# open-speech/HTK

Hardware: AMD Instinct MI355X
Metric: herest_gmm_frame_state_loglik_per_sec (higher is better)
Workload: dtype f32 (scores: bf16x3 split operands, fp32 accumulate) + f64 (alpha / beta with fp32-transcendental log-add, accumulators); 1 GPU; HERest EM iteration (pass + accumulator all-reduce + model update), 5000 tied states x 16 mix, D=39, 1250 x 500-frame utterances per GPU (BASELINE config[2]: 10k utterances sharded 8-way); states=5000, mix=16, utts_per_gpu=1250, frames=500, chunks=1, update=HERest -m 3 -v 0.01, on the device

## Files before the change

### htk_amd/csrc/fb.hip

```cpp
#include <hip/hip_runtime.h>
#include <cstdio>
#include <cstdlib>
#include <cstring>
#include <cmath>
#include <algorithm>
#include <vector>
#include <thread>
#include <mutex>
#include <condition_variable>
#include <functional>
#include "internal.h"
#include "hipcheck.h"
#include "kernels.h"
#include "devbuf.h"

static constexpr char fbOwner[] = "fb";
typedef DevBufT<fbOwner> DevBuf;

struct PrepPool {
   std::vector<std::thread> th;
   std::mutex mu;
   std::condition_variable cvGo, cvDone;
   std::function<void(int)> job;
   int generation = 0, pending = 0, nJobs = 0;
// ... 105 lines not shown

struct ResLayout {
   size_t nUtt;
   size_t status() const { return sizeof(double) * nUtt; }
   size_t counter() const { return (sizeof(double) + sizeof(int)) * nUtt; }
   size_t flag() const { return counter() + sizeof(int); } size_t bytes() const { return counter() + 2 * sizeof(int); }
};

enum { UTT_NO_TEE = 1, UTT_ALL_LR = 2 };

struct htkamd_fb : BatchTables {
   htkamd_model *m = nullptr;
   int nUtt = 0;
   int debug = 0;
   int forceGeneral = 0;
   int noStatePath = 0;
   int noLrPath = 0;
   int topoVersion = 0;
   std::vector<unsigned char> uttFlags;
   UttClasses cls;
   size_t gamTotal = 0, betaWTotal = 0, alphaWTotal = 0;
   int totalFrames = 0, nCellsMax = 1, QMax = 1, TMax = 1, blockDim = 64;
   long long frameStates = 0;
   const float *dX = nullptr;
   DevBuf d_arena;
   DevBuf d_qLo, d_qHi, d_aLo, d_aHi, d_outp, d_beta, d_gam, d_alpha, d_pr;
   DevBuf d_betaW;
   DevBuf d_tmE, d_tmMaxP;
   DevBuf d_outpU;
   DevBuf d_alphaW, d_qBeam, d_aBeam, d_trPart, d_hits, d_hitCtl;
   DevBuf d_sink;
   DevBuf d_stCnt, d_stBucket;
   DevBuf d_laneRec;
   bool mixStateLast = false;
   bool mixDeferred = false;
   FbArgs *faMix = nullptr;
   const int *qBeamLast = nullptr;
   DevBuf d_transOff, d_trOccOff, d_counter;
   DevBuf d_rec, d_recSorted, d_recCtl;
   int recCapForce = 0;
   PrepPool *pool = nullptr; std::vector<PrepChunk> *chunks = nullptr;
   void *h_arena = nullptr; size_t h_arenaCap = 0;
   void *h_res = nullptr; size_t h_resCap = 0;
   hipEvent_t evRes = nullptr; bool resPending = false;
   bool f16Pass = false;
   hipEvent_t ev[6] = {}, evK[2] = {}, evCopy = nullptr;
   hipStream_t resStream = nullptr;
   bool timed = false, copyPending = false, scored = false;
   int evMode = 0, evModeLast = 0;
   ResLayout res() const { return {(size_t)nUtt}; }
};

static bool compat_revisit(const htkamd_model *m) { return (m->compat & HTKAMD_COMPAT_STREAM_REVISIT) && m->NSt > 1 && m->NSt != 3 && !m->tiedMix; }

extern "C" int htkamd_fb_create(htkamd_model *m, htkamd_fb **out)
{
   if (!m || !out) { htkamd_set_error("fb_create: NULL argument"); return HTKAMD_EINVAL; }
   if (m->fullc) { htkamd_set_error("fb_create: forward-backward on FULLC models is not supported yet (its mixture statistics are diagonal)"); return HTKAMD_EMODEL; }
   if (m->maxM > 4096) { htkamd_set_error("fb_create: %d mixture components per state not supported", m->maxM); return HTKAMD_EMODEL; }
   htkamd_fb *fb = new htkamd_fb();
   fb->m = m;
   auto fail = [&](const char *what, hipError_t e) { htkamd_set_error("fb_create: %s: %s", what, hipGetErrorString(e)); htkamd_fb_destroy(fb); return HTKAMD_EHIP; };
   hipError_t e;
   for (hipEvent_t *v : {&fb->ev[0], &fb->ev[1], &fb->ev[2], &fb->ev[3], &fb->ev[4], &fb->ev[5], &fb->evK[0], &fb->evK[1]})
      if ((e = hipEventCreate(v)) != hipSuccess) return fail("hipEventCreate", e);
   if ((e = hipEventCreateWithFlags(&fb->evCopy, hipEventDisableTiming)) != hipSuccess) return fail("hipEventCreate", e);
// ... 424 lines not shown
   fa.mN = fb->mN.dev; fa.mTp = fb->mTp.dev; fa.mCell0 = fb->mCell0.dev; fa.mSlot0 = fb->mSlot0.dev; fa.mDms = fb->mDms.dev; fa.mHmm = fb->mHmm.dev; fa.mTrans = fb->mTrans.dev;
   fa.sQ = fb->sQ.dev; fa.thrCell = fb->thrCell.dev; fa.cQ = fb->cQ.dev; fa.cI = fb->cI.dev; fa.slotState = fb->slotState.dev;
   fa.taperLo = fb->taperLo.dev; fa.taperHi = fb->taperHi.dev;
   fa.qLo = (short *)fb->d_qLo.p; fa.qHi = (short *)fb->d_qHi.p; fa.aLo = (short *)fb->d_aLo.p; fa.aHi = (short *)fb->d_aHi.p;
   fa.X = fb->dX; fa.transP = m->d_transP; fa.outp = (float *)fb->d_outp.p;
   fa.beta = (double *)fb->d_beta.p; fa.gam = (double *)fb->d_gam.p; fa.alphaDbg = fb->debug ? (double *)fb->d_alpha.p : nullptr;
   fa.pr = (double *)fb->d_pr.p; fa.status = (int *)((char *)fb->d_pr.p + fb->res().status());
   fa.stateCompOff = m->d_stateCompOff; fa.compGauss = m->d_compGauss;
   fa.NSt = m->NSt; fa.outpU = (const float *)fb->d_outpU.p; fa.dimStream = m->d_dimStream;
   fa.compatRevisit = compat_revisit(m) && !fb->nextSame.empty(); fa.nextSame = fb->nextSame.dev;
   fa.transOff = (const int *)fb->d_transOff.p; fa.trOccOff = (const int *)fb->d_trOccOff.p;
   fa.compLogWt = m->d_compLogWt; fa.gparam = m->d_gparam; fa.mean = m->d_mean; fa.laddTab = m->d_laddTab;
   fa.PS = m->PS; fa.D = m->D; fa.maxN = m->maxN; fa.maxM = m->maxM;
   fa.nCellsMax = fb->nCellsMax; fa.QMax = fb->QMax; fa.TMax = fb->TMax;
   fa.acc = accs->d_vec; fa.lay = accs->lay;
   fa.pruneInit = cfg->pruneInit; fa.pruneInc = cfg->pruneInc; fa.pruneLim = cfg->pruneLim;
   fa.minLogExp = m->minLogExp; fa.minFrwdP = cfg->minFrwdP; fa.uFlags = cfg->uFlags;
   fa.gamTotal = fb->gamTotal; fa.gamOffByUtt = fb->gamOff.dev; fa.gamChunkUtt = fb->gamChunkUtt.dev;
   return fa;
}

struct LdsSizes { size_t beta, alpha; };
static LdsSizes fb_lds_sizes(const FbArgs &fa)
{
   const size_t nc = fa.nCellsMax, qm = fa.QMax + 3, mn = fa.maxN, tm = (size_t)fa.TMax + 3;
   auto r8 = [](size_t x) { return (x + 7) & ~(size_t)7; };
   const size_t ldsTab = r8((size_t)LADD_NK * (LADD_DEG + 1) * 8);
   return {2 * r8(nc * 8) + r8(qm * 8) + r8(nc * mn * 4) + 4 * r8(qm * 4) + r8(32) + ldsTab,
           2 * r8(nc * 8) + r8(3 * nc * 8) + r8(qm * 8) + r8(nc * (mn + 1) * 8) + ldsTab + r8(3 * nc * 4) + 2 * r8(nc * mn * 4) + 4 * r8(qm * 4) + 2 * r8(tm * 2)};
}

static const int clsW[4] = {1, 2, 4, 8};

static int fb_reserve_lr(htkamd_fb *fb, const htkamd_fb_config *cfg, FbArgs &fa, bool fastLadd, hipStream_t s)
{
   const htkamd_model *m = fb->m;
   int rc;
   size_t rows = 0;
   for (int W : clsW) rows += (size_t)fb->cls.of(FB_LEFT_TO_RIGHT, W).n * htkamd_stats_lr_chunks(fb->TMax) * W;
   const size_t nfr = fb->totalFrames ? fb->totalFrames : 1;
   if ((rc = fb->d_laneRec.reserve(sizeof(LaneRec) * (fb->slotState.size() + 1))) || (rc = fb->d_sink.reserve(256))) return rc;
   fa.laneRec = (LaneRec *)fb->d_laneRec.p; fa.sink = (double *)fb->d_sink.p;
   if ((rc = fb->d_alphaW.reserve(sizeof(double) * (fb->alphaWTotal + 64))) || (rc = fb->d_qBeam.reserve(sizeof(int) * (nfr + 2))) ||
       (rc = fb->d_aBeam.reserve(sizeof(int) * (nfr + 2))) || (rc = fb->d_trPart.reserve(sizeof(double) * htkamd_stats_lr_row_doubles() * (rows + 256))) ||
       (rc = fb->d_hits.reserve(sizeof(MixHit) * (rows * htkamd_stats_lr_region_cap() + 64))) || (rc = fb->d_hitCtl.reserve(sizeof(int) * (rows + 1))))
      return rc;
   fa.alphaW = (double *)fb->d_alphaW.p; fa.qBeam = (int *)fb->d_qBeam.p; fa.aBeam = (int *)fb->d_aBeam.p; fa.trPart = (double *)fb->d_trPart.p;
   fa.hits = (MixHit *)fb->d_hits.p; fa.hitCtl = (int *)fb->d_hitCtl.p; fa.nHitRegions = (int)rows; fa.hitRegionCap = htkamd_stats_lr_region_cap();
   fa.hitSlots = (m->NSt > 1 || m->tiedMix) ? 1 : 0;
   fa.qBeamNP = fb->qBeamNP.dev;
   if (htkamd_beta_lr_is_lean(fa, fastLadd)) fa.qBeam = const_cast<int *>(fb->qBeamNP.dev);
   fb->qBeamLast = fa.qBeam;
   fb->mixStateLast = false;
   fa.fastMath = fastLadd ? 1 : 0;
   if (fb->recCapForce == 0 && !fa.hitSlots && m->maxM <= 16 && (m->D == 39 || m->D == 26 || m->D == 13) &&
       (cfg->uFlags & (HTKAMD_UPMEANS | HTKAMD_UPVARS | HTKAMD_UPMIXES))) {
      size_t cap = 64;
      while (cap < 65536 && cap * (size_t)m->S < (size_t)16 * fb->totalFrames) cap <<= 1;
      while (cap > 64 && cap * (size_t)m->S * sizeof(HitS) > ((size_t)1 << 30)) cap >>= 1;
      { const char *e = getenv("HTKAMD_ST_CAP"); if (e && atoi(e) > 0) cap = (size_t)atoi(e); }
      if ((rc = fb->d_stCnt.reserve(sizeof(int) * (3 * (size_t)m->S + 4))) || (rc = fb->d_stBucket.reserve(sizeof(HitS) * cap * (size_t)m->S))) return rc;
      fb->mixStateLast = true;
      fa.stCnt = (int *)fb->d_stCnt.p; fa.nTiedStates = m->S; fa.stBucket = (HitS *)fb->d_stBucket.p; fa.stCap = (int)cap;
      HIPCHECK(hipMemsetAsync(fa.stCnt, 0, sizeof(int) * (3 * (size_t)m->S + 4), s));
   }
   return HTKAMD_OK;
}

struct FamilyKernels { int family; int (*beta)(const FbArgs &, int, bool, hipStream_t); int (*alpha)(const FbArgs &, int, bool, hipStream_t); };
static const FamilyKernels familyKernels[] = {{FB_LANE_PER_MODEL, htkamd_launch_beta_w, htkamd_launch_alpha_w},
                                              {FB_LANE_PER_STATE, htkamd_launch_beta_s, htkamd_launch_alpha_s},
                                              {FB_LEFT_TO_RIGHT, htkamd_launch_beta_lr, htkamd_launch_alpha_lr}};

static int fb_recursions(htkamd_fb *fb, const FbArgs &fa, const LdsSizes &lds, bool fastLadd, bool noEv, hipStream_t s)
{
   int rc;
   for (int pass = 0; pass < 2; pass++) {
      FbArgs fc = fa;
      const UttClasses::Range g = fb->cls.general();
      fc.uttList = fb->uttList.dev + g.first; fc.nList = g.n;
      if (g.n > 0 && (rc = pass == 0 ? htkamd_launch_beta(fc, fb->blockDim, lds.beta, s) : htkamd_launch_alpha(fc, fb->blockDim, lds.alpha, s))) return rc;
      for (const FamilyKernels &k : familyKernels)
         for (int c = 3; c >= 0; c--) {
            const UttClasses::Range r = fb->cls.of(k.family, clsW[c]);
            fc.uttList = fb->uttList.dev + r.first; fc.nList = r.n;
            if ((rc = (pass == 0 ? k.beta : k.alpha)(fc, clsW[c], fastLadd, s))) return rc;
         }
      if (!noEv) HIPCHECK(hipEventRecord(fb->ev[2 + pass], s));
   }
   return HTKAMD_OK;
}

static int fb_stats_lr(htkamd_fb *fb, const FbArgs &fa, bool fastLadd, bool noEv, hipStream_t s)
{
   int rc;
   FbArgs fc = fa;
   size_t rowOff = 0;
// ... 20 lines not shown
      if ((rc = fb->d_rec.reserve(sizeof(MixRec) * cap)) || (rc = fb->d_recSorted.reserve(sizeof(MixRec) * cap)) ||
          (rc = fb->d_recCtl.reserve(sizeof(int) * (3 * ((size_t)m->G + 1) + 1 + (size_t)m->G / 2048 + 2))))
         return rc;
      fa.rec = (MixRec *)fb->d_rec.p; fa.recSorted = (MixRec *)fb->d_recSorted.p; fa.recCap = (int)cap; fa.G = m->G; fa.recCtl = (int *)fb->d_recCtl.p;
   }
   if (m->tiedMix || m->NSt > 1) {
      fa.stateCompOff = m->d_stateCompOff; fa.rec = nullptr;
      if (fb->nUtt > nLr && (rc = m->tiedMix ? htkamd_launch_mixstats_tm(fa, s) : htkamd_launch_mixstats_ms(fa, s))) return rc;
      if (nLr > 0 && (rc = htkamd_launch_mixhits_streams(fa, m->tiedMix != 0, s))) return rc;
      return HTKAMD_OK;
   }
   const bool dense = fb->nUtt > nLr && fa.gamTotal > 0, listed = nLr > 0;
   if ((rc = htkamd_launch_mixstats(fa, s, dense, listed, defer))) return rc;
   if (defer && listed && !dense && htkamd_mixstate_applies(fa)) {
      if (!fb->faMix) fb->faMix = new FbArgs();
      *fb->faMix = fa;
      fb->mixDeferred = true;
   }
   return HTKAMD_OK;
}

static int fb_execute_impl(htkamd_fb *fb, const htkamd_fb_config *cfg, htkamd_accs *accs, void *stream, bool defer)
{
   if (!fb || !cfg || !accs) { htkamd_set_error("fb_execute: NULL argument"); return HTKAMD_EINVAL; }
   fb->mixDeferred = false;
   if (accs->m != fb->m) { htkamd_set_error("fb_execute: accumulators belong to a different model"); return HTKAMD_EINVAL; }
   if (fb->nUtt == 0) return HTKAMD_OK;
   const htkamd_model *m = fb->m;
   hipStream_t s = (hipStream_t)stream;
   if (fb->topoVersion != m->topoVersion) {
      htkamd_set_error("fb_execute: the model's minimum durations changed since htkamd_fb_prepare (a re-estimated transition reached or left zero): prepare the batch again");
      return HTKAMD_EINVAL;
   }
   const ScoreArgs sa = fb_score_args(fb, cfg);
   if (cfg->scoreMode & ~(HTKAMD_SCORE_MFMA | HTKAMD_SCORE_FASTLADD | HTKAMD_SCORE_BF16 | HTKAMD_SCORE_F16 | HTKAMD_SCORE_SOUTP)) { htkamd_set_error("fb_execute: unknown score mode %d", cfg->scoreMode); return HTKAMD_EINVAL; }
   const bool fastLadd = (cfg->scoreMode & HTKAMD_SCORE_FASTLADD) != 0;
   FbArgs fa = fb_args(fb, cfg, accs);
   const LdsSizes lds = fb_lds_sizes(fa);

   int rc;
   if (fb->copyPending) HIPCHECK(hipStreamWaitEvent(s, fb->evCopy, 0));
   const bool noEv = fb->evMode == 1;
   HIPCHECK(hipEventRecord(fb->ev[0], s));
   if (m->tiedMix) {
      fa.tmE = (float *)fb->d_tmE.p; fa.tmMaxP = (float *)fb->d_tmMaxP.p; fa.tmPoolOff = m->d_tmPoolOff; fa.tmPool = m->tmPool; fa.totalFrames = fb->totalFrames;
      fa.tmTasks = fb->tasks.dev; fa.tmNTasks = (int)fb->tasks.size(); fa.tmSlotState = sa.slotState; fa.tmOut = sa.out;
      fa.compWeight = m->d_compWeight; fa.var = m->d_var;
      if ((rc = htkamd_launch_tm_score(fa, s))) return rc;
      fb->scored = false;
   } else {
      if ((rc = htkamd_launch_score(cfg->scoreMode, m, sa, s, fb->evK[0], fb->evK[1]))) return rc;
      fb->scored = sa.nTasks > 0;
   }
   if (m->NSt > 1) {
      if ((rc = htkamd_launch_combine_streams(fa, s))) return rc;
      if (m->maxM > 1) fa.stateCompOff = m->d_msCompOff;
   } else if (m->tiedMix) fa.stateCompOff = m->d_msCompOff;
   if (!noEv) HIPCHECK(hipEventRecord(fb->ev[1], s));
   if (fb->cls.nGeneral() > 0 && lds.alpha > 160 * 1024) { htkamd_set_error("fb_execute: %zu bytes of LDS needed (max model size %zu states)", lds.alpha, (size_t)m->maxN); return HTKAMD_EMODEL; }
   if ((rc = fb->d_betaW.reserve(sizeof(double) * (fb->betaWTotal + 8 * 512)))) return rc;
   fa.betaW = (double *)fb->d_betaW.p;
   if (fb->cls.nLr() > 0 && (rc = fb_reserve_lr(fb, cfg, fa, fastLadd, s))) return rc;
   if ((rc = fb_recursions(fb, fa, lds, fastLadd, noEv, s)) || (rc = fb_stats_lr(fb, fa, fastLadd, noEv, s)) || (rc = fb_mix_stats(fb, cfg, fa, defer, s))) return rc;
   HIPCHECK(hipEventRecord(fb->ev[5], s));
   fb->timed = true; fb->evModeLast = noEv ? 1 : 0;
   return HTKAMD_OK;
}

extern "C" int htkamd_fb_execute(htkamd_fb *fb, const htkamd_fb_config *cfg, htkamd_accs *accs, void *stream)
{
   return fb_execute_impl(fb, cfg, accs, stream, false);
}

extern "C" int htkamd_fb_execute_begin(htkamd_fb *fb, const htkamd_fb_config *cfg, htkamd_accs *accs, void *stream, int *deferred)
{
   if (deferred) *deferred = 0;
   const int rc = fb_execute_impl(fb, cfg, accs, stream, true);
   if (rc == HTKAMD_OK && deferred && fb && fb->nUtt > 0) *deferred = fb->mixDeferred ? 1 : 0;
   return rc;
}

extern "C" int htkamd_fb_execute_mix(htkamd_fb *fb, int state0, int state1, void *stream)
{
   if (!fb) { htkamd_set_error("fb_execute_mix: NULL"); return HTKAMD_EINVAL; }
   if (fb->nUtt == 0 || !fb->mixDeferred) return HTKAMD_OK;
   const int rc = htkamd_launch_mixstate_range(*fb->faMix, state0, state1, (hipStream_t)stream);
   if (rc) return rc;
   HIPCHECK(hipEventRecord(fb->ev[5], (hipStream_t)stream));
   return HTKAMD_OK;
}


static int res_staging(htkamd_fb *fb, size_t bytes)
{
   if (bytes > fb->h_resCap) {
      if (fb->h_res) (void)hipHostFree(fb->h_res);
      fb->h_res = nullptr; fb->h_resCap = 0;
// ... 193 lines not shown
```

### htk_amd/csrc/fb_kernels.hip

```cpp
#include <hip/hip_runtime.h>
#include <cstring>
#include <cstdlib>
#include "internal.h"
#include "hipcheck.h"
#include "kernels.h"
#include "ladd.h"

#define ladd(x, y, mle) ladd_tab((x), (y), (mle), ltab)

#define EXPFLOOR (-100.0)

struct CellMeta {
   int q, i, N, mc0, ms0;
};

struct LdsCarve {
   char *p;
   __device__ explicit LdsCarve(void *base) : p((char *)base) {}
   template <typename T> __device__ T *take(size_t n)
   {
      T *r = (T *)p;
      p += ((n * sizeof(T) + 7) & ~(size_t)7);
      return r;
   }
// ... 865 lines not shown
                  const int fr = __shfl(mine.frame, ii);
                  Lv[e] = (i + e < nb) ? __shfl(mine.L, ii) : 0.0;
                  xv[e] = (k < D) ? a.X[(size_t)fr * D + k] : 0.0f;
               }
#pragma unroll
               for (int e = 0; e < 4; e++) {
                  if (i + e >= nb) break;
                  const float z = xv[e] - mean;
                  const double L = Lv[e];
                  if (upMu && upVa) {
                     const float zl = (float)((double)z * L);
                     sMu += (double)zl; sVa += (double)(z * zl);
                  } else if (upMu) sMu += (double)z * L;
                  else if (upVa) sVa += (double)(z * z) * L;
               }
            }
         }
         if (k < D) {
            if (upMu && sMu != 0.0) atomicAdd(a.acc + a.lay.mu + (size_t)g * D + k, sMu);
            if (upVa && sVa != 0.0) atomicAdd(a.acc + a.lay.va + (size_t)g * D + k, sVa);
         }
         if (k0 == 0) {
#pragma unroll
            for (int o = 32; o > 0; o >>= 1) sL += __shfl_xor(sL, o);
            if (lane == 0) {
               if (upMu) atomicAdd(a.acc + a.lay.muOcc + g, sL);
               if (upVa) atomicAdd(a.acc + a.lay.vaOcc + g, sL);
            }
         }
      }
   }
}

#define MS_EU 8
template <int DT, int MODE>
__global__ __launch_bounds__(64, MS_EU) void k_mixstate(FbArgs a)
{
#define MS_CHUNK 32
#define MS_CAP 128
#define MS_PARTS 4
   constexpr int GS = 16, HPS = 64 / GS, NQ = (DT + 1) / 2, XS = (DT + 3) & ~3;
   constexpr int CH = MS_CHUNK;
   __shared__ float xs[CH * XS];
   __shared__ double Lt[CH][GS];
   __shared__ double hSeed[CH];
   const int st = a.stBase + blockIdx.x, lane = threadIdx.x, grp = lane / GS, sub = lane % GS;
   const int nst = a.stCnt[st] < a.stCap ? a.stCnt[st] : a.stCap;
   const int part = blockIdx.y;
   const int r0 = part * MS_CAP, r1 = (part == (int)gridDim.y - 1 || r0 + MS_CAP > nst) ? nst : r0 + MS_CAP;
   if (r0 >= nst) return;
   const HitS *bucket = a.stBucket + (size_t)st * a.stCap;
   const int c0 = a.stateCompOff[st], M = a.stateCompOff[st + 1] - c0;
   const bool single = (M == 1 || a.maxM == 1);
   constexpr bool upMu = (MODE & 1) != 0, upVa = (MODE & 2) != 0;
   const bool upWt = a.uFlags & HTKAMD_UPMIXES;
   __shared__ float4 pl[NQ][GS];
   int g = 0;
   float wt = 0.0f, gcst = 0.0f;
   if (sub < M) {
      g = a.compGauss[c0 + sub];
      wt = a.compLogWt[c0 + sub];
      gcst = a.gparam[(size_t)g * a.PS + 2 * DT];
      if (grp == 0) {
         const float4 *P4 = (const float4 *)(a.gparam + (size_t)g * a.PS);
#pragma unroll
         for (int q = 0; q < NQ; q++) { const float4 pv = P4[q]; pl[q][sub] = make_float4(pv.x, pv.z, pv.y, pv.w); }
      }
   }
   float meanR[GS];
   const int gOfLane = (lane < M) ? a.compGauss[c0 + lane] : 0;
#pragma unroll
   for (int m = 0; m < GS; m++) { const int gm_ = __builtin_amdgcn_readlane(gOfLane, m); meanR[m] = (m < M && lane < DT) ? a.mean[(size_t)gm_ * DT + lane] : 0.0f; }
   double sMu[GS], sVa[GS];
#pragma unroll
   for (int m = 0; m < GS; m++) { sMu[m] = 0.0; sVa[m] = 0.0; }
   double wtAcc = 0.0;
   int nTriples = 0;
   const double minF = uniform_f64((double)a.minFrwdP);

   for (int base = r0; base < r1; base += CH) {
      const int n = (r1 - base < CH) ? r1 - base : CH;
      __syncthreads();
      int hfr = 0;
// ... 66 lines not shown
                     xv[i] = xs[h * XS + (lane < DT ? lane : 0)];
                  }
#pragma unroll
                  for (int i = 0; i < 4; i++) {
                     const double L = Lv[i];
                     const float z = xv[i] - mean;
                     if constexpr (upMu && upVa) { const float zl = (float)((double)z * L); mu += (double)zl; va += (double)(z * zl); }
                     else if constexpr (upMu) mu += (double)z * L;
                     else va += (double)(z * z) * L;
                  }
               }
               sMu[m] = mu; sVa[m] = va;
            }
         }
      }
   }
#pragma unroll
   for (int m = 0; m < GS; m++) {
      if (m < M && lane < DT) {
         const int gm = a.compGauss[c0 + m];
         if (upMu && sMu[m] != 0.0) atomicAdd(a.acc + a.lay.mu + (size_t)gm * DT + lane, sMu[m]);
         if (upVa && sVa[m] != 0.0) atomicAdd(a.acc + a.lay.va + (size_t)gm * DT + lane, sVa[m]);
      }
   }
   double w = wtAcc;
   w += __shfl_xor(w, 16); w += __shfl_xor(w, 32);
   if (grp == 0 && sub < M && w != 0.0) {
      if (upWt) atomicAdd(a.acc + a.lay.wt + c0 + sub, w);
      if (upMu) atomicAdd(a.acc + a.lay.muOcc + g, w);
      if (upVa) atomicAdd(a.acc + a.lay.vaOcc + g, w);
   }
#pragma unroll
   for (int o = 32; o > 0; o >>= 1) nTriples += __shfl_xor(nTriples, o);
   if (lane == 0) { if (part == 0) a.stCnt[a.nTiedStates + 4 + 2 * st] = nst; atomicAdd(a.stCnt + a.nTiedStates + 5 + 2 * st, nTriples); }
   double so = (sub < M) ? w : 0.0;
#pragma unroll
   for (int o = GS / 2; o > 0; o >>= 1) so += __shfl_xor(so, o);
   if (lane == 0 && so != 0.0) atomicAdd(a.acc + a.lay.wtOcc + st, so);
}

bool htkamd_mixstate_applies(const FbArgs &a) { return a.stCnt && a.stBucket && !a.hitSlots && a.maxM <= 16 && (a.D == 39 || a.D == 26 || a.D == 13); }
int htkamd_launch_mixstate_range(const FbArgs &a_in, int st0, int st1, hipStream_t s)
{
   if (st0 < 0 || st1 > a_in.nTiedStates || st0 > st1) { htkamd_set_error("mixture statistics: state range [%d, %d) outside the set's %d", st0, st1, a_in.nTiedStates); return HTKAMD_EINVAL; }
   if (st0 == st1) return HTKAMD_OK;
   FbArgs a = a_in;
   a.stBase = st0;
   const int S = st1 - st0;
   const int mode = ((a.uFlags & HTKAMD_UPMEANS) ? 1 : 0) | ((a.uFlags & HTKAMD_UPVARS) ? 2 : 0);
#define MS_LAUNCH(DT_) \
   do { \
      if (mode == 3) hipLaunchKernelGGL((k_mixstate<DT_, 3>), dim3(S, MS_PARTS), dim3(64), 0, s, a); \
      else if (mode == 1) hipLaunchKernelGGL((k_mixstate<DT_, 1>), dim3(S, MS_PARTS), dim3(64), 0, s, a); \
      else if (mode == 2) hipLaunchKernelGGL((k_mixstate<DT_, 2>), dim3(S, MS_PARTS), dim3(64), 0, s, a); \
      else hipLaunchKernelGGL((k_mixstate<DT_, 0>), dim3(S, MS_PARTS), dim3(64), 0, s, a); \
   } while (0)
   if (a.D == 39) MS_LAUNCH(39); else if (a.D == 26) MS_LAUNCH(26); else MS_LAUNCH(13);
#undef MS_LAUNCH
   HIPCHECK(hipGetLastError());
   return HTKAMD_OK;
}

static int set_lds_limit(const void *fn, size_t lds)
{
   if (lds > 64 * 1024)
      HIPCHECK(hipFuncSetAttribute(fn, hipFuncAttributeMaxDynamicSharedMemorySize, (int)lds));
   return HTKAMD_OK;
}

int htkamd_launch_beta(const FbArgs &a, int blockDim, size_t lds, hipStream_t s)
{
   int rc = set_lds_limit((const void *)k_beta, lds);
   if (rc) return rc;
   hipLaunchKernelGGL(k_beta, dim3(a.nList), dim3(blockDim), lds, s, a);
   HIPCHECK(hipGetLastError());
   return HTKAMD_OK;
}

int htkamd_launch_alpha(const FbArgs &a, int blockDim, size_t lds, hipStream_t s)
{
   int rc = set_lds_limit((const void *)k_alpha, lds);
   if (rc) return rc;
   hipLaunchKernelGGL(k_alpha, dim3(a.nList), dim3(blockDim), lds, s, a);
   HIPCHECK(hipGetLastError());
   return HTKAMD_OK;
}

int htkamd_launch_mixstats(const FbArgs &a_in, hipStream_t s, bool dense, bool listed, bool deferState)
// ... 427 lines not shown
```

### htk_amd/csrc/fb_lr.hip

```cpp
#include <hip/hip_runtime.h>
#include <type_traits>
#include "internal.h"
#include "hipcheck.h"
#include "kernels.h"
#include "ladd.h"
#include "wavegrp.h"
#include "fb_state.h"

typedef const __attribute__((address_space(4))) int cint_lr;

#define ALPHA_S(t) (a.alphaW[ud.alphaW0 + (size_t)((t) - 1) * L + gl])
#define ALPHA_E(t, q_) (a.alphaW[ud.alphaW0 + (size_t)T * L + (size_t)((t) - 1) * ud.QP + ((q_) - 1)])

struct LrRegs {
   int q, j, N, mi;
   bool first, last;
   float aSelf, aNext, aPrev;
   float aEntry, aExit;
   float aExitPrev, aEntryNext;
};

__device__ __forceinline__ void load_lr(LrRegs &s, const FbArgs &a, const UttDesc &ud, int gl, bool valid)
{
   s.q = 0; s.j = 2; s.N = 3; s.mi = 0; s.first = false; s.last = false;
// ... 378 lines not shown
         hi0 = hi1; lo1 = lo2; hi1 = hi2; lo2 = w3 & 0xffff; hi2 = has2 ? (w3 >> 16) : 0;
         fLo0 = fLo1;
         if (lo1 != lo1Of) { fLo1 = flOf[lo1]; lo1Of = lo1; }
         if (hi1 != hi1Of) { fHi1 = flOf[hi1 > 0 ? hi1 : 1]; hi1Of = hi1; }
         { const int e0 = ((hi0 < Q) ? hi0 + 1 : hi0) + 1; if (e0 != e0Of) { fE0 = flOf[e0]; e0Of = e0; } }
         if (fLo0 != mLoOf) { mLo = MaskW<W>::range(fLo0, L - 1); mLoOf = fLo0; }
         if (fE0 != mEOf) { mE = MaskW<W>::range(0, fE0 - 1); mEOf = fE0; }
         wSame = (has2 && wq1 == wq2 && wq2 == w3) ? w3 : -1;
         wq1 = wq2; wq2 = w3;
      }
      return true;
   };
   if (T >= 1 && step(1, std::true_type{}, std::false_type{})) {
      int t = 2;
      for (; t + 2 <= T; t++) if (!step(t, std::false_type{}, std::true_type{})) { t = T + 1; break; }
      for (; t <= T; t++) if (!step(t, std::false_type{}, std::false_type{})) break;
   }

   if (err) {
      if (gl == 0) { a.status[u] = HTKAMD_UTT_EALPHA; atomicAdd(a.acc + a.lay.nUttSkipped, 1.0); }
      return;
   }
   if (valid && s.first) atomicAdd(a.acc + a.lay.nEgs + cHmm, 1.0);
   if (gl == 0) {
      atomicAdd(a.acc + a.lay.totalPr, pr);
      atomicAdd(a.acc + a.lay.totalT, (double)T);
      atomicAdd(a.acc + a.lay.nUttDone, 1.0);
      atomicAdd(a.acc + a.lay.nEval, (double)ud.nEval);
   }
#undef ladd
}

#define STATS_FC 32
#define TR_ROW 16
#define EXP_TERM(acc, x) do { if constexpr (FAST) acc += exp_fast(x); else if ((x) > EXPFLOOR) acc += exp_tab((x), etab); } while (0)

__global__ __launch_bounds__(256) void k_trans_reduce(FbArgs a, int nRows)
{
   __shared__ double sh[256][TR_ROW + 1];
   __shared__ int mixed;
   const int tid = threadIdx.x, r = blockIdx.x * 256 + tid;
   if (tid == 0) mixed = 0;
   const double *row = a.trPart + (size_t)r * TR_ROW;
   int ti = -1;
   if (r < nRows) ti = (int)row[TR_ROW - 1];
#pragma unroll
   for (int k = 0; k < 11; k++) sh[tid][k] = (ti >= 0) ? row[k] : 0.0;
   __syncthreads();
   __shared__ int tiBlock;
   if (tid == 0) tiBlock = -1;
   __syncthreads();
   if (ti >= 0) atomicMax(&tiBlock, ti);
   __syncthreads();
   const int tb = tiBlock;
   if (ti >= 0 && ti != tb) mixed = 1;
   __syncthreads();
   auto add_row = [&](int t_, const double *v) {
      const int N0 = a.trOccOff[t_ + 1] - a.trOccOff[t_];
      double *tr = a.acc + a.lay.tr + a.transOff[t_];
      double *oc = a.acc + a.lay.trOcc + a.trOccOff[t_];
      for (int i = 2; i <= 4 && i <= N0 - 1; i++) {
         if (v[i - 2] != 0.0) atomicAdd(tr + (size_t)(i - 1) * N0 + (i - 1), v[i - 2]);
         if (v[3 + i - 2] != 0.0) atomicAdd(tr + (size_t)(i - 1) * N0 + i, v[3 + i - 2]);
         if (v[7 + i - 2] != 0.0) atomicAdd(oc + (i - 1), v[7 + i - 2]);
      }
      if (v[6] != 0.0) atomicAdd(tr + 1, v[6]);
      if (v[10] != 0.0) atomicAdd(oc, v[10]);
   };
   if (tb < 0) return;
   if (mixed) {
      if (ti >= 0) add_row(ti, sh[tid]);
      return;
   }
   const int k = tid & 15, part = tid >> 4;
   double v = 0.0;
   if (k < 11) for (int rr = part; rr < 256; rr += 16) v += sh[rr][k];
   __syncthreads();
   sh[part][k] = v;
   __syncthreads();
   if (tid < 11) {
      double tot = 0.0;
      for (int p = 0; p < 16; p++) tot += sh[p][tid];
      sh[16][tid] = tot;
   }
   __syncthreads();
   if (tid == 0) add_row(tb, sh[16]);
}

#include "fb_lr_lean.inc"

template <bool FAST> static void launch_beta_lr(const FbArgs &a, int W, hipStream_t s)
{
   if (W == 1) hipLaunchKernelGGL((k_beta_lr<1, FAST>), dim3(a.nList), dim3(64), 0, s, a);
   else if (W == 2) hipLaunchKernelGGL((k_beta_lr<2, FAST>), dim3(a.nList), dim3(128), 0, s, a);
   else if (W == 4) hipLaunchKernelGGL((k_beta_lr<4, FAST>), dim3(a.nList), dim3(256), 0, s, a);
   else hipLaunchKernelGGL((k_beta_lr<8, FAST>), dim3(a.nList), dim3(512), 0, s, a);
}
static void launch_alpha_lr(const FbArgs &a, int W, hipStream_t s)
{
   if (W == 1) hipLaunchKernelGGL((k_alpha_lr<1>), dim3(a.nList), dim3(64), 0, s, a);
   else if (W == 2) hipLaunchKernelGGL((k_alpha_lr<2>), dim3(a.nList), dim3(128), 0, s, a);
// ... 24 lines not shown
int htkamd_launch_beta_lr(const FbArgs &a, int W, bool fast, hipStream_t s)
{
   if (a.nList <= 0) return HTKAMD_OK;
   if (htkamd_beta_lr_is_lean(a, fast)) {
      const dim3 grid(a.nList);
      if (W == 2) hipLaunchKernelGGL(k_beta_np2, grid, dim3(64), 0, s, a);
      else if (W == 1) hipLaunchKernelGGL((k_beta_np<1>), grid, dim3(64), 0, s, a);
      else if (W == 4) hipLaunchKernelGGL((k_beta_np<4>), grid, dim3(256), 0, s, a);
      else hipLaunchKernelGGL((k_beta_np<8>), grid, dim3(512), 0, s, a);
      HIPCHECK(hipGetLastError());
      return HTKAMD_OK;
   }
   if (fast) launch_beta_lr<true>(a, W, s); else launch_beta_lr<false>(a, W, s);
   HIPCHECK(hipGetLastError());
   return HTKAMD_OK;
}

int htkamd_launch_alpha_lr(const FbArgs &a, int W, bool fast, hipStream_t s)
{
   if (a.nList <= 0) return HTKAMD_OK;
   if (!fast) launch_alpha_lr(a, W, s);
   else if (a.alphaDbg) launch_alpha_f<true>(a, W, s);
   else launch_alpha_f<false>(a, W, s);
   HIPCHECK(hipGetLastError());
   return HTKAMD_OK;
}

int htkamd_launch_stats_lr(const FbArgs &a, int W, bool fast, hipStream_t s)
{
   if (a.nList <= 0) return HTKAMD_OK;
   const int nChunks = htkamd_stats_lr_chunks(a.TMax);
   if (fast) launch_stats_sp<true>(a, W, nChunks, s); else launch_stats_sp<false>(a, W, nChunks, s);
   const int nRows = a.nList * nChunks * W;
   hipLaunchKernelGGL(k_trans_reduce, dim3((nRows + 255) / 256), dim3(256), 0, s, a, nRows);
   HIPCHECK(hipGetLastError());
   return HTKAMD_OK;
}
```

### htk_amd/csrc/gmm_bf16.hip

```cpp
#include <hip/hip_runtime.h>
#include <hip/hip_ext.h>
#include "internal.h"
#include "hipcheck.h"
#include "kernels.h"

typedef float f4 __attribute__((ext_vector_type(4)));
typedef float f4u __attribute__((ext_vector_type(4), aligned(4)));
typedef __bf16 bf8 __attribute__((ext_vector_type(8)));
typedef unsigned int u4 __attribute__((ext_vector_type(4)));
typedef const __attribute__((address_space(4))) int cint;

#define EXP2(x) __builtin_amdgcn_exp2f(x)
#define LOG2(x) __builtin_amdgcn_logf(x)
#define B16_COL_TILES 2

__device__ __forceinline__ float rows_max_b(float v)
{
   auto a = __builtin_amdgcn_permlane16_swap(__float_as_uint(v), __float_as_uint(v), false, false);
   v = fmaxf(__uint_as_float(a[0]), __uint_as_float(a[1]));
   auto b = __builtin_amdgcn_permlane32_swap(__float_as_uint(v), __float_as_uint(v), false, false);
   return fmaxf(__uint_as_float(b[0]), __uint_as_float(b[1]));
}
__device__ __forceinline__ float rows_sum_b(float v)
{
// ... 431 lines not shown
               if (3 * ks + 1 < 18) lse_slice(3 * ks + 1);
               Cc = __builtin_amdgcn_mfma_f32_32x32x16_bf16(wa[ks][0], zb[ks][1], Cc, 0, 0, 0);
               Cc = __builtin_amdgcn_mfma_f32_32x32x16_bf16(wa[ks][1], zb[ks][0], Cc, 0, 0, 0);
               if (3 * ks + 2 < 18) lse_slice(3 * ks + 2);
               Cx = __builtin_amdgcn_mfma_f32_32x32x16_bf16(wa[ks][0], zb[ks][0], Cx, 0, 0, 0);
            }
            for (int sl = 3 * KS; sl < 18; sl++) lse_slice(sl);
            asm volatile("" : "+v"(resP));
            resQ = resP; oQ = oPrev; haveQ = prevAct;
#pragma unroll
            for (int b = 0; b < 4; b++) {
               const f4 ci = __builtin_bit_cast(f4, wbuf[buf][KS * 192 + kh * 4 + b]);
#pragma unroll
               for (int r = 0; r < 4; r++) yP[4 * b + r] = (Cx[4 * b + r] + Cc[4 * b + r]) + ci[r];
            }
         }
         prevAct = actJ; oPrev += oStep;
         asm volatile("s_waitcnt vmcnt(0)" ::: "memory");
         __syncthreads();
         buf ^= 1;
      }
      if (haveQ) { if (fw + fcol < tk.nFrames) *oQ = resQ; }
      if (prevAct) {
         const float res = lse_full();
         if (fw + fcol < tk.nFrames && 2 * (nPairs - 1) + kh < tk.nSlots) *oPrev = res;
      }
   }
}

int htkamd_launch_score_bf16(const htkamd_model *m, const ScoreArgs &a, hipStream_t stream, hipEvent_t evStart, hipEvent_t evStop)
{
   if (a.nTasks <= 0) return HTKAMD_OK;
   { const int rc = htkamd_model_table_current(m, HTKAMD_SCORE_BF16, stream); if (rc) return rc; }
   if (a.qCounters == a.taskCounter + 8) HIPCHECK(hipMemsetAsync(a.taskCounter, 0, 16 * sizeof(int), stream));
   else {
      HIPCHECK(hipMemsetAsync(a.taskCounter, 0, sizeof(int), stream));
      if (a.qCounters) HIPCHECK(hipMemsetAsync(a.qCounters, 0, 8 * sizeof(int), stream));
   }
   if (m->f16Wide && (size_t)m->nTiles * ((size_t)3 * m->bf16NC * 64 * 16 + 64 * 16) >= ((size_t)1 << 32)) {
      htkamd_set_error("score_bf16: a table of %d tiles is beyond the kernel's 32-bit staging offsets", m->nTiles); return HTKAMD_EMODEL;
   }
   if (m->f16Wide) {
      dim3 block(256);
#define W_LAUNCH(KS_) do { const int b_ = a.nTasks < 256 * b16w_eu(KS_) ? a.nTasks : 256 * b16w_eu(KS_); \
                           hipExtLaunchKernelGGL((k_score_bf16w<KS_>), dim3(b_), block, 0, stream, evStart, evStop, 0, a); } while (0)
      if (m->bf16Dense) {
         W_LAUNCH(5); HIPCHECK(hipGetLastError());
         return HTKAMD_OK;
      }
      switch (m->bf16NC) {
      case 3: W_LAUNCH(6); break;
      case 2: W_LAUNCH(4); break;
      case 1: W_LAUNCH(2); break;
      default: htkamd_set_error("score_bf16: no kernel for %d K-chunks", m->bf16NC); return HTKAMD_EMODEL;
      }
#undef W_LAUNCH
      HIPCHECK(hipGetLastError());
      return HTKAMD_OK;
   }
   const int parts = B16_TASK_FRAMES / (16 * B16_COL_TILES * B16_WPB);
   int blocks = a.nTasks * parts;
   if (blocks > 256 * ((B16_COL_TILES > 2 ? 8 : 12) / B16_WPB)) blocks = 256 * ((B16_COL_TILES > 2 ? 8 : 12) / B16_WPB);
   dim3 grid(blocks), block(64 * B16_WPB);
   switch (m->bf16NC) {
   case 3: hipExtLaunchKernelGGL((k_score_bf16<3>), grid, block, 0, stream, evStart, evStop, 0, a); break;
   case 2: hipExtLaunchKernelGGL((k_score_bf16<2>), grid, block, 0, stream, evStart, evStop, 0, a); break;
   case 1: hipExtLaunchKernelGGL((k_score_bf16<1>), grid, block, 0, stream, evStart, evStop, 0, a); break;
// ... 156 lines not shown
```

### htk_amd/csrc/kernels.h

```cpp
#ifndef HTKAMD_KERNELS_H
#define HTKAMD_KERNELS_H
#include <hip/hip_runtime.h>
#include <vector>
#include "internal.h"

#define SCORE_TILE_FRAMES 128
#define B16_TASK_FRAMES 128
#define SCORE_TASK_SLOTS  16
#define SCORE_TASK_SLOTS_WIDE 64
#define SCORE_TASK_SLOTS_EXACT 8

struct ScoreTask {
   int frame0;
   int nFrames;
   int slot0;
   int nSlots;
   int outSlot0;
   int ldo;
   size_t outBase;
};

struct ScoreArgs {
   const ScoreTask *tasks = nullptr;
   int nTasks = 0;
   const float *X = nullptr;
   const int *slotState = nullptr;
   float *out = nullptr;
   const int *stateCompOff = nullptr, *compGauss = nullptr;
   const float *compLogWt = nullptr, *gparam = nullptr;
   int PS = 0, D = 0;
   double minLogExp = 0.0;
   const double *laddTab = nullptr;
   int *taskCounter = nullptr;
   const float *mfmaTab = nullptr;
   const int *stateTileOff = nullptr;
   const void *bf16Tab = nullptr;
   const void *f16Tab = nullptr;
   const int *f16Ctl = nullptr;
   int *rangeFlag = nullptr;
   const float *var = nullptr;
   int NSt = 1;
   const float *streamWt = nullptr;
   const int *qStart = nullptr;
   int *qCounters = nullptr;
   const int *slotRange = nullptr;
};

static inline ScoreArgs htkamd_score_args(const htkamd_model *m)
{
   ScoreArgs a;
   a.stateCompOff = m->d_stateCompOff; a.compGauss = m->d_compGauss; a.compLogWt = m->d_compLogWt;
   a.gparam = m->d_gparam; a.PS = m->PS; a.D = m->D; a.minLogExp = m->minLogExp; a.laddTab = m->d_laddTab;
   a.mfmaTab = m->d_mfmaTab; a.stateTileOff = m->d_stateTileOff; a.bf16Tab = m->d_bf16Tab; a.var = m->d_var;
   a.NSt = m->NSt; a.streamWt = m->d_streamWt;
   return a;
}

static inline int htkamd_tile_count(int T, int nSlots, int FR, int SL) { return ((T + FR - 1) / FR) * ((nSlots + SL - 1) / SL); }
static inline void htkamd_tile_tasks(ScoreTask *tk, int frame0, int T, int slot0, int nSlots, size_t outBase, int ldo, int FR, int SL)
{
   for (int t0 = 0; t0 < T; t0 += FR)
      for (int k0 = 0; k0 < nSlots; k0 += SL, tk++) {
         tk->frame0 = frame0 + t0; tk->nFrames = (T - t0 < FR) ? T - t0 : FR;
         tk->slot0 = slot0 + k0; tk->nSlots = (nSlots - k0 < SL) ? nSlots - k0 : SL;
         tk->outSlot0 = k0; tk->ldo = ldo; tk->outBase = outBase + (size_t)t0;
      }
}
static inline void htkamd_tile_tasks(std::vector<ScoreTask> &v, int frame0, int T, int slot0, int nSlots, size_t outBase, int ldo, int FR, int SL)
{
   if (T <= 0 || nSlots <= 0) return;
   const size_t n = v.size();
   v.resize(n + (size_t)htkamd_tile_count(T, nSlots, FR, SL));
   htkamd_tile_tasks(v.data() + n, frame0, T, slot0, nSlots, outBase, ldo, FR, SL);
}

int htkamd_launch_score_exact(const htkamd_model *m, const ScoreArgs &a, hipStream_t stream, hipEvent_t evStart = nullptr, hipEvent_t evStop = nullptr, bool soutp = false, bool diagc = false);
int htkamd_launch_score_full(const htkamd_model *m, const ScoreArgs &a, hipStream_t stream, hipEvent_t evStart, hipEvent_t evStop, bool soutp, bool diagc);
int htkamd_launch_score_mfma(const htkamd_model *m, const ScoreArgs &a, hipStream_t stream, hipEvent_t evStart = nullptr, hipEvent_t evStop = nullptr);
// ... 68 lines not shown
   int nCellsMax, QMax, TMax;
   double *acc;
   htkamd_accs_layout lay;
   double pruneInit, pruneInc, pruneLim, minLogExp;
   float minFrwdP;
   int uFlags;
   size_t gamTotal;
   const size_t *gamOffByUtt;
   const int *gamChunkUtt;
   MixRec *rec, *recSorted;
   int recCap, G;
   int *recCtl;
   int NSt;
   const float *outpU;
   int compatRevisit;
   const int *nextSame;
   const int *dimStream;
   float *tmE;
   float *tmMaxP;
   const int *tmPoolOff;
   int tmPool, totalFrames;
   const ScoreTask *tmTasks; int tmNTasks; const int *tmSlotState; float *tmOut;
   const float *compWeight, *var;
   int tmCombine;
   const float *streamWt;
   MixHit *hits;
   int hitSlots;
   int *hitCtl;
   int nHitRegions, hitRegionCap;
   LaneRec *laneRec;
   const int *qBeamNP;
   int stBase;
   int *stCnt; int nTiedStates; HitS *stBucket; int stCap;
   int fastMath;
   double *sink;
};

int htkamd_launch_beta(const FbArgs &a, int blockDim, size_t lds, hipStream_t s);
int htkamd_launch_alpha(const FbArgs &a, int blockDim, size_t lds, hipStream_t s);
int htkamd_launch_mixstats(const FbArgs &a, hipStream_t s, bool dense, bool listed, bool deferState = false);
bool htkamd_mixstate_applies(const FbArgs &a);
int htkamd_launch_mixstate_range(const FbArgs &a, int st0, int st1, hipStream_t s);
int htkamd_launch_combine_streams(const FbArgs &a, hipStream_t s);
int htkamd_launch_mixstats_ms(const FbArgs &a, hipStream_t s);
int htkamd_launch_tm_score(const FbArgs &a, hipStream_t s);
int htkamd_launch_mixstats_tm(const FbArgs &a, hipStream_t s);
int htkamd_launch_mixhits_streams(const FbArgs &a, bool tied, hipStream_t s);
int htkamd_tm_score_block(const htkamd_model *m, const ScoreArgs &sa, int nRows, float tmBeam, hipStream_t s);
int htkamd_launch_beta_s(const FbArgs &a, int W, bool fast, hipStream_t s);
int htkamd_launch_alpha_s(const FbArgs &a, int W, bool fast, hipStream_t s);
int htkamd_launch_beta_w(const FbArgs &a, int W, bool fast, hipStream_t s);
int htkamd_launch_beta_lr(const FbArgs &a, int W, bool fast, hipStream_t s);
bool htkamd_beta_lr_is_lean(const FbArgs &a, bool fast);
int htkamd_launch_alpha_lr(const FbArgs &a, int W, bool fast, hipStream_t s);
int htkamd_launch_stats_lr(const FbArgs &a, int W, bool fast, hipStream_t s);
int htkamd_stats_lr_chunks(int TMax);
size_t htkamd_stats_lr_row_doubles(void);
int htkamd_stats_lr_region_cap(void);
int htkamd_launch_alpha_w(const FbArgs &a, int W, bool fast, hipStream_t s);

#endif
```

Baseline: 29.29 billion frame-state log-lik/s.

## Self-reset mixstate counters and fold transition reduce into mixstate launch

The mixstate kernel now clears its per-state counters and the score task counters itself, using an arrival counter so the last part of each state resets its slot. This removes the hipMemsetAsync calls on later iterations when the buffers are known to be clean. It also folds the k_trans_reduce work into extra blocks of the mixstate grid, which saves one kernel launch. It skips the ev[0] event record when events are disabled. The cost is added atomics and host-side tracking of which buffers are clean across calls. That tracking is fragile if a call aborts partway.

```diff
diff --git a/htk_amd/csrc/fb.hip b/htk_amd/csrc/fb.hip
--- a/htk_amd/csrc/fb.hip
+++ b/htk_amd/csrc/fb.hip
@@ -161,6 +161,7 @@
    DevBuf d_sink;
    DevBuf d_stCnt, d_stBucket;
    DevBuf d_laneRec;
+   const void *scoreCtlClean = nullptr, *stCntClean = nullptr; size_t stCntCleanCap = 0;
    bool mixStateLast = false;
    bool mixDeferred = false;
    FbArgs *faMix = nullptr;
@@ -651,7 +652,14 @@
 
 static const int clsW[4] = {1, 2, 4, 8};
 
-static int fb_reserve_lr(htkamd_fb *fb, const htkamd_fb_config *cfg, FbArgs &fa, bool fastLadd, hipStream_t s)
+static bool fb_mixstate_pass(const htkamd_fb *fb, const htkamd_fb_config *cfg)
+{
+   const htkamd_model *m = fb->m;
+   return fb->recCapForce == 0 && m->NSt == 1 && !m->tiedMix && m->maxM <= 16 && (m->D == 39 || m->D == 26 || m->D == 13) &&
+          (cfg->uFlags & (HTKAMD_UPMEANS | HTKAMD_UPVARS | HTKAMD_UPMIXES));
+}
+
+static int fb_reserve_lr(htkamd_fb *fb, const htkamd_fb_config *cfg, FbArgs &fa, bool fastLadd, const void *stCntWasClean, hipStream_t s)
 {
    const htkamd_model *m = fb->m;
    int rc;
@@ -672,16 +680,16 @@
    fb->qBeamLast = fa.qBeam;
    fb->mixStateLast = false;
    fa.fastMath = fastLadd ? 1 : 0;
-   if (fb->recCapForce == 0 && !fa.hitSlots && m->maxM <= 16 && (m->D == 39 || m->D == 26 || m->D == 13) &&
-       (cfg->uFlags & (HTKAMD_UPMEANS | HTKAMD_UPVARS | HTKAMD_UPMIXES))) {
+   if (fb_mixstate_pass(fb, cfg)) {
       size_t cap = 64;
       while (cap < 65536 && cap * (size_t)m->S < (size_t)16 * fb->totalFrames) cap <<= 1;
       while (cap > 64 && cap * (size_t)m->S * sizeof(HitS) > ((size_t)1 << 30)) cap >>= 1;
-      { const char *e = getenv("HTKAMD_ST_CAP"); if (e && atoi(e) > 0) cap = (size_t)atoi(e); }
-      if ((rc = fb->d_stCnt.reserve(sizeof(int) * (3 * (size_t)m->S + 4))) || (rc = fb->d_stBucket.reserve(sizeof(HitS) * cap * (size_t)m->S))) return rc;
+      { const char *e = getenv("HTKAMD_ST_CAP"); if (e && atoi(e) > 0) cap = std::min<size_t>((size_t)atoi(e), 65536); }
+      const size_t ctlBytes = sizeof(int) * (4 * (size_t)m->S + 4);
+      if ((rc = fb->d_stCnt.reserve(ctlBytes)) || (rc = fb->d_stBucket.reserve(sizeof(HitS) * cap * (size_t)m->S))) return rc;
       fb->mixStateLast = true;
       fa.stCnt = (int *)fb->d_stCnt.p; fa.nTiedStates = m->S; fa.stBucket = (HitS *)fb->d_stBucket.p; fa.stCap = (int)cap;
-      HIPCHECK(hipMemsetAsync(fa.stCnt, 0, sizeof(int) * (3 * (size_t)m->S + 4), s));
+      if (!(fa.msSelfReset && stCntWasClean == fb->d_stCnt.p && fb->stCntCleanCap == fb->d_stCnt.cap)) HIPCHECK(hipMemsetAsync(fa.stCnt, 0, ctlBytes, s));
    }
    return HTKAMD_OK;
 }
@@ -768,16 +776,27 @@
       htkamd_set_error("fb_execute: the model's minimum durations changed since htkamd_fb_prepare (a re-estimated transition reached or left zero): prepare the batch again");
       return HTKAMD_EINVAL;
    }
-   const ScoreArgs sa = fb_score_args(fb, cfg);
+   ScoreArgs sa = fb_score_args(fb, cfg);
    if (cfg->scoreMode & ~(HTKAMD_SCORE_MFMA | HTKAMD_SCORE_FASTLADD | HTKAMD_SCORE_BF16 | HTKAMD_SCORE_F16 | HTKAMD_SCORE_SOUTP)) { htkamd_set_error("fb_execute: unknown score mode %d", cfg->scoreMode); return HTKAMD_EINVAL; }
    const bool fastLadd = (cfg->scoreMode & HTKAMD_SCORE_FASTLADD) != 0;
    FbArgs fa = fb_args(fb, cfg, accs);
    const LdsSizes lds = fb_lds_sizes(fa);
+   const bool selfReset = !defer && fb->cls.nLr() == fb->nUtt && fb_mixstate_pass(fb, cfg);
+   const void *scoreWasClean = fb->scoreCtlClean, *stCntWasClean = fb->stCntClean;
+   fb->scoreCtlClean = fb->stCntClean = nullptr;
+   if (selfReset) {
+      size_t rows = 0;
+      for (int W : clsW) rows += (size_t)fb->cls.of(FB_LEFT_TO_RIGHT, W).n * htkamd_stats_lr_chunks(fb->TMax) * W;
+      fa.msSelfReset = 1; fa.scoreCtl = (int *)fb->d_counter.p;
+      fa.foldRows = (cfg->uFlags & HTKAMD_UPTRANS) ? (int)rows : 0;
+      fa.msExtra = fa.foldRows > 0 ? (fa.foldRows + 255) / 256 : 1;
+      sa.countersZero = scoreWasClean == fb->d_counter.p;
+   }
 
    int rc;
    if (fb->copyPending) HIPCHECK(hipStreamWaitEvent(s, fb->evCopy, 0));
    const bool noEv = fb->evMode == 1;
-   HIPCHECK(hipEventRecord(fb->ev[0], s));
+   if (!noEv) HIPCHECK(hipEventRecord(fb->ev[0], s));
    if (m->tiedMix) {
       fa.tmE = (float *)fb->d_tmE.p; fa.tmMaxP = (float *)fb->d_tmMaxP.p; fa.tmPoolOff = m->d_tmPoolOff; fa.tmPool = m->tmPool; fa.totalFrames = fb->totalFrames;
       fa.tmTasks = fb->tasks.dev; fa.tmNTasks = (int)fb->tasks.size(); fa.tmSlotState = sa.slotState; fa.tmOut = sa.out;
@@ -796,9 +815,10 @@
    if (fb->cls.nGeneral() > 0 && lds.alpha > 160 * 1024) { htkamd_set_error("fb_execute: %zu bytes of LDS needed (max model size %zu states)", lds.alpha, (size_t)m->maxN); return HTKAMD_EMODEL; }
    if ((rc = fb->d_betaW.reserve(sizeof(double) * (fb->betaWTotal + 8 * 512)))) return rc;
    fa.betaW = (double *)fb->d_betaW.p;
-   if (fb->cls.nLr() > 0 && (rc = fb_reserve_lr(fb, cfg, fa, fastLadd, s))) return rc;
+   if (fb->cls.nLr() > 0 && (rc = fb_reserve_lr(fb, cfg, fa, fastLadd, stCntWasClean, s))) return rc;
    if ((rc = fb_recursions(fb, fa, lds, fastLadd, noEv, s)) || (rc = fb_stats_lr(fb, fa, fastLadd, noEv, s)) || (rc = fb_mix_stats(fb, cfg, fa, defer, s))) return rc;
    HIPCHECK(hipEventRecord(fb->ev[5], s));
+   if (selfReset) { fb->scoreCtlClean = fb->d_counter.p; fb->stCntClean = fb->d_stCnt.p; fb->stCntCleanCap = fb->d_stCnt.cap; }
    fb->timed = true; fb->evModeLast = noEv ? 1 : 0;
    return HTKAMD_OK;
 }
diff --git a/htk_amd/csrc/fb_kernels.hip b/htk_amd/csrc/fb_kernels.hip
--- a/htk_amd/csrc/fb_kernels.hip
+++ b/htk_amd/csrc/fb_kernels.hip
@@ -921,6 +921,62 @@
    }
 }
 
+__device__ __forceinline__ void mixstate_arrive(const FbArgs &a, int st, int nst, int nTriples, int nParts)
+{
+   const int S = a.nTiedStates;
+   int *word = a.stCnt + 3 * S + 4 + st;
+   const int old = atomicAdd(word, (1 << 28) | nTriples);
+   if ((old >> 28) != nParts - 1) return;
+   a.stCnt[S + 4 + 2 * st] = nst; a.stCnt[S + 5 + 2 * st] = (old & 0x0fffffff) + nTriples;
+   a.stCnt[st] = 0; *word = 0;
+}
+
+__device__ __forceinline__ void mixstate_extra(const FbArgs &a, int b, int tid)
+{
+   if (b == 0 && a.msSelfReset) {
+      if (tid < 16 && a.scoreCtl) a.scoreCtl[tid] = 0;
+      if (tid == 16) a.stCnt[a.nTiedStates] = 0;
+   }
+   int ti[4], tb = -1;
+#pragma unroll
+   for (int i = 0; i < 4; i++) {
+      const int r = b * 256 + i * 64 + tid;
+      ti[i] = (r < a.foldRows) ? (int)a.trPart[(size_t)r * TR_ROW + TR_ROW - 1] : -1;
+      tb = ti[i] > tb ? ti[i] : tb;
+   }
+#pragma unroll
+   for (int o = 32; o > 0; o >>= 1) { const int v = __shfl_xor(tb, o); tb = v > tb ? v : tb; }
+   if (tb < 0) return;
+   bool odd = false;
+#pragma unroll
+   for (int i = 0; i < 4; i++) odd = odd || (ti[i] >= 0 && ti[i] != tb);
+   const bool mixed = __any(odd);
+   double v[11];
+#pragma unroll
+   for (int k = 0; k < 11; k++) v[k] = 0.0;
+#pragma unroll
+   for (int i = 0; i < 4; i++) {
+      if (ti[i] < 0) continue;
+      const double *row = a.trPart + (size_t)(b * 256 + i * 64 + tid) * TR_ROW;
+      if (mixed) {
+         double w[11];
+#pragma unroll
+         for (int k = 0; k < 11; k++) w[k] = row[k];
+         trans_add_row(a, ti[i], w);
+      } else {
+#pragma unroll
+         for (int k = 0; k < 11; k++) v[k] += row[k];
+      }
+   }
+   if (mixed) return;
+#pragma unroll
+   for (int k = 0; k < 11; k++) {
+#pragma unroll
+      for (int o = 32; o > 0; o >>= 1) v[k] += __shfl_xor(v[k], o);
+   }
+   if (tid == 0) trans_add_row(a, tb, v);
+}
+
 #define MS_EU 8
 template <int DT, int MODE>
 __global__ __launch_bounds__(64, MS_EU) void k_mixstate(FbArgs a)
@@ -933,11 +989,15 @@
    __shared__ float xs[CH * XS];
    __shared__ double Lt[CH][GS];
    __shared__ double hSeed[CH];
-   const int st = a.stBase + blockIdx.x, lane = threadIdx.x, grp = lane / GS, sub = lane % GS;
+   if ((int)blockIdx.x < a.msExtra) {
+      if (blockIdx.y == 0) mixstate_extra(a, (int)blockIdx.x, (int)threadIdx.x);
+      return;
+   }
+   const int st = a.stBase + (int)blockIdx.x - a.msExtra, lane = threadIdx.x, grp = lane / GS, sub = lane % GS;
    const int nst = a.stCnt[st] < a.stCap ? a.stCnt[st] : a.stCap;
    const int part = blockIdx.y;
    const int r0 = part * MS_CAP, r1 = (part == (int)gridDim.y - 1 || r0 + MS_CAP > nst) ? nst : r0 + MS_CAP;
-   if (r0 >= nst) return;
+   if (r0 >= nst) { if (a.msSelfReset && lane == 0) mixstate_arrive(a, st, nst, 0, (int)gridDim.y); return; }
    const HitS *bucket = a.stBucket + (size_t)st * a.stCap;
    const int c0 = a.stateCompOff[st], M = a.stateCompOff[st + 1] - c0;
    const bool single = (M == 1 || a.maxM == 1);
@@ -1070,7 +1130,10 @@
    }
 #pragma unroll
    for (int o = 32; o > 0; o >>= 1) nTriples += __shfl_xor(nTriples, o);
-   if (lane == 0) { if (part == 0) a.stCnt[a.nTiedStates + 4 + 2 * st] = nst; atomicAdd(a.stCnt + a.nTiedStates + 5 + 2 * st, nTriples); }
+   if (lane == 0) {
+      if (a.msSelfReset) mixstate_arrive(a, st, nst, nTriples, (int)gridDim.y);
+      else { if (part == 0) a.stCnt[a.nTiedStates + 4 + 2 * st] = nst; atomicAdd(a.stCnt + a.nTiedStates + 5 + 2 * st, nTriples); }
+   }
    double so = (sub < M) ? w : 0.0;
 #pragma unroll
    for (int o = GS / 2; o > 0; o >>= 1) so += __shfl_xor(so, o);
@@ -1088,10 +1151,10 @@
    const int mode = ((a.uFlags & HTKAMD_UPMEANS) ? 1 : 0) | ((a.uFlags & HTKAMD_UPVARS) ? 2 : 0);
 #define MS_LAUNCH(DT_) \
    do { \
-      if (mode == 3) hipLaunchKernelGGL((k_mixstate<DT_, 3>), dim3(S, MS_PARTS), dim3(64), 0, s, a); \
-      else if (mode == 1) hipLaunchKernelGGL((k_mixstate<DT_, 1>), dim3(S, MS_PARTS), dim3(64), 0, s, a); \
-      else if (mode == 2) hipLaunchKernelGGL((k_mixstate<DT_, 2>), dim3(S, MS_PARTS), dim3(64), 0, s, a); \
-      else hipLaunchKernelGGL((k_mixstate<DT_, 0>), dim3(S, MS_PARTS), dim3(64), 0, s, a); \
+      if (mode == 3) hipLaunchKernelGGL((k_mixstate<DT_, 3>), dim3(S + a.msExtra, MS_PARTS), dim3(64), 0, s, a); \
+      else if (mode == 1) hipLaunchKernelGGL((k_mixstate<DT_, 1>), dim3(S + a.msExtra, MS_PARTS), dim3(64), 0, s, a); \
+      else if (mode == 2) hipLaunchKernelGGL((k_mixstate<DT_, 2>), dim3(S + a.msExtra, MS_PARTS), dim3(64), 0, s, a); \
+      else hipLaunchKernelGGL((k_mixstate<DT_, 0>), dim3(S + a.msExtra, MS_PARTS), dim3(64), 0, s, a); \
    } while (0)
    if (a.D == 39) MS_LAUNCH(39); else if (a.D == 26) MS_LAUNCH(26); else MS_LAUNCH(13);
 #undef MS_LAUNCH
diff --git a/htk_amd/csrc/fb_lr.hip b/htk_amd/csrc/fb_lr.hip
--- a/htk_amd/csrc/fb_lr.hip
+++ b/htk_amd/csrc/fb_lr.hip
@@ -434,7 +434,6 @@
 }
 
 #define STATS_FC 32
-#define TR_ROW 16
 #define EXP_TERM(acc, x) do { if constexpr (FAST) acc += exp_fast(x); else if ((x) > EXPFLOOR) acc += exp_tab((x), etab); } while (0)
 
 __global__ __launch_bounds__(256) void k_trans_reduce(FbArgs a, int nRows)
@@ -457,18 +456,7 @@
    const int tb = tiBlock;
    if (ti >= 0 && ti != tb) mixed = 1;
    __syncthreads();
-   auto add_row = [&](int t_, const double *v) {
-      const int N0 = a.trOccOff[t_ + 1] - a.trOccOff[t_];
-      double *tr = a.acc + a.lay.tr + a.transOff[t_];
-      double *oc = a.acc + a.lay.trOcc + a.trOccOff[t_];
-      for (int i = 2; i <= 4 && i <= N0 - 1; i++) {
-         if (v[i - 2] != 0.0) atomicAdd(tr + (size_t)(i - 1) * N0 + (i - 1), v[i - 2]);
-         if (v[3 + i - 2] != 0.0) atomicAdd(tr + (size_t)(i - 1) * N0 + i, v[3 + i - 2]);
-         if (v[7 + i - 2] != 0.0) atomicAdd(oc + (i - 1), v[7 + i - 2]);
-      }
-      if (v[6] != 0.0) atomicAdd(tr + 1, v[6]);
-      if (v[10] != 0.0) atomicAdd(oc, v[10]);
-   };
+   auto add_row = [&](int t_, const double *v) { trans_add_row(a, t_, v); };
    if (tb < 0) return;
    if (mixed) {
       if (ti >= 0) add_row(ti, sh[tid]);
@@ -559,6 +547,7 @@
    const int nChunks = htkamd_stats_lr_chunks(a.TMax);
    if (fast) launch_stats_sp<true>(a, W, nChunks, s); else launch_stats_sp<false>(a, W, nChunks, s);
    const int nRows = a.nList * nChunks * W;
+   if (a.foldRows > 0) { HIPCHECK(hipGetLastError()); return HTKAMD_OK; }
    hipLaunchKernelGGL(k_trans_reduce, dim3((nRows + 255) / 256), dim3(256), 0, s, a, nRows);
    HIPCHECK(hipGetLastError());
    return HTKAMD_OK;
diff --git a/htk_amd/csrc/gmm_bf16.hip b/htk_amd/csrc/gmm_bf16.hip
--- a/htk_amd/csrc/gmm_bf16.hip
+++ b/htk_amd/csrc/gmm_bf16.hip
@@ -487,7 +487,7 @@
 {
    if (a.nTasks <= 0) return HTKAMD_OK;
    { const int rc = htkamd_model_table_current(m, HTKAMD_SCORE_BF16, stream); if (rc) return rc; }
-   if (a.qCounters == a.taskCounter + 8) HIPCHECK(hipMemsetAsync(a.taskCounter, 0, 16 * sizeof(int), stream));
+   if (a.qCounters == a.taskCounter + 8) { if (!a.countersZero) HIPCHECK(hipMemsetAsync(a.taskCounter, 0, 16 * sizeof(int), stream)); }
    else {
       HIPCHECK(hipMemsetAsync(a.taskCounter, 0, sizeof(int), stream));
       if (a.qCounters) HIPCHECK(hipMemsetAsync(a.qCounters, 0, 8 * sizeof(int), stream));
diff --git a/htk_amd/csrc/kernels.h b/htk_amd/csrc/kernels.h
--- a/htk_amd/csrc/kernels.h
+++ b/htk_amd/csrc/kernels.h
@@ -44,6 +44,7 @@
    const int *qStart = nullptr;
    int *qCounters = nullptr;
    const int *slotRange = nullptr;
+   bool countersZero = false;
 };
 
 static inline ScoreArgs htkamd_score_args(const htkamd_model *m)
@@ -178,9 +179,28 @@
    const int *qBeamNP;
    int stBase;
    int *stCnt; int nTiedStates; HitS *stBucket; int stCap;
+   int msSelfReset, msExtra, foldRows;
+   int *scoreCtl;
    int fastMath;
    double *sink;
 };
+
+#define TR_ROW 16
+#ifdef __HIPCC__
+__device__ __forceinline__ void trans_add_row(const FbArgs &a, int t_, const double *v)
+{
+   const int N0 = a.trOccOff[t_ + 1] - a.trOccOff[t_];
+   double *tr = a.acc + a.lay.tr + a.transOff[t_];
+   double *oc = a.acc + a.lay.trOcc + a.trOccOff[t_];
+   for (int i = 2; i <= 4 && i <= N0 - 1; i++) {
+      if (v[i - 2] != 0.0) atomicAdd(tr + (size_t)(i - 1) * N0 + (i - 1), v[i - 2]);
+      if (v[3 + i - 2] != 0.0) atomicAdd(tr + (size_t)(i - 1) * N0 + i, v[3 + i - 2]);
+      if (v[7 + i - 2] != 0.0) atomicAdd(oc + (i - 1), v[7 + i - 2]);
+   }
+   if (v[6] != 0.0) atomicAdd(tr + 1, v[6]);
+   if (v[10] != 0.0) atomicAdd(oc, v[10]);
+}
+#endif
 
 int htkamd_launch_beta(const FbArgs &a, int blockDim, size_t lds, hipStream_t s);
 int htkamd_launch_alpha(const FbArgs &a, int blockDim, size_t lds, hipStream_t s);
```

Result: no change. 29.39 billion frame-state log-lik/s, median of 4 (+0.4%).
